# MIT-SPARK/TEASER-plusplus

Measured on AMD Instinct MI355X. Metric: registrations/sec at N=10000 correspondences, 95% outliers, higher is better.
Workload: dtype bf16x3-split MFMA + f32 filter with FP64 fix-up for K1 (bitmap bit-identical to FP64); f64 estimators

## Files before the change

teaser-plusplus_amd/csrc/kernels_graph.hip:

```cpp
#include <algorithm>
#include <utility>
#include <vector>

#include <cstdio>
#include <cstdlib>

#include "internal.h"
#include "fixup_item.h"
#include "fixup_regions.h"
#include "k1_consts.h"
#include "wave_utils.h"

namespace thip {

struct EdgeConst {
  double beta;
  double beta2;
  double m2beta2;
  double beta4;
  double s_hat;
};

__device__ __forceinline__ bool tim_edge_exact(double ax, double ay, double az, double bx,
                                               double by, double bz, double beta) {
// ... 316 lines not shown
    const float na = (float)na_d, nb = (float)nb_d;
    int ra, rb, pa, pb;
    k1c::xy_shifts(kexp, &ra, &rb, &pa, &pb);
    const float fra = (float)k1c::pow2_d(-ra), frb = (float)k1c::pow2_d(-rb), fpa = (float)k1c::pow2_d(-pa);
    const unsigned short P = f16_bits((float)k1c::pow2_d(-pb));
    unsigned short A[32], B[32];
    for (int k = 0; k < 32; ++k) A[k] = B[k] = 0;
    const float cs[3] = {sx, sy, sz}, cd[3] = {dx, dy, dz};
    float h, m, l;
    for (int c = 0; c < 3; ++c) {
      f16_split3(cs[c] * fra, &h, &m, &l);
      A[3 * c] = f16_bits(h); A[3 * c + 1] = A[3 * c]; A[3 * c + 2] = f16_bits(m);
      f16_split3(cs[c] * frb, &h, &m, &l);
      B[3 * c] = f16_bits(2.0f * h); B[3 * c + 1] = f16_bits(2.0f * m); B[3 * c + 2] = B[3 * c];
      f16_split3(cd[c] * fra, &h, &m, &l);
      A[16 + 3 * c] = f16_bits(h); A[16 + 3 * c + 1] = A[16 + 3 * c]; A[16 + 3 * c + 2] = f16_bits(m);
      f16_split3(cd[c] * frb, &h, &m, &l);
      B[16 + 3 * c] = f16_bits(-2.0f * h); B[16 + 3 * c + 1] = f16_bits(-2.0f * m); B[16 + 3 * c + 2] = B[16 + 3 * c];
    }
    f16_split3(na * fpa, &h, &m, &l);
    A[9] = f16_bits(-h); A[10] = f16_bits(-m); A[11] = f16_bits(-l); B[9] = P; B[10] = P; B[11] = P;
    B[12] = A[9]; B[13] = A[10]; B[14] = A[11]; A[12] = P; A[13] = P; A[14] = P;
    f16_split3(nb * fpa, &h, &m, &l);
    A[25] = f16_bits(h); A[26] = f16_bits(m); A[27] = f16_bits(l); B[25] = P; B[26] = P; B[27] = P;
    B[28] = A[25]; B[29] = A[26]; B[30] = A[27]; A[28] = P; A[29] = P; A[30] = P;
    A[31] = 0xb400;
    B[31] = 0x3c00;
    TimOperandTile2* tile = ops + d.w_off + (ip >> 6);
    const int gq = (ip >> 5) & 1, cc = ip & 31;
    for (int mf = 0; mf < kTimRowOperands; ++mf)
      for (int hh = 0; hh < 2; ++hh) {
        const unsigned short* pa = A + 16 * mf + 8 * hh;
        tile->a[gq][mf][hh][cc] = make_uint4(pa[0] | ((unsigned int)pa[1] << 16), pa[2] | ((unsigned int)pa[3] << 16),
                                             pa[4] | ((unsigned int)pa[5] << 16), pa[6] | ((unsigned int)pa[7] << 16));
        if (mf >= kTimColOperands) continue;
        const unsigned short* pb = B + 16 * mf + 8 * hh;
        tile->b[gq][mf][hh][cc] = make_uint4(pb[0] | ((unsigned int)pb[1] << 16), pb[2] | ((unsigned int)pb[3] << 16),
                                             pb[4] | ((unsigned int)pb[5] << 16), pb[6] | ((unsigned int)pb[7] << 16));
      }
    mx = na > nb ? na : nb;
    if (!(mx == mx)) mx = INFINITY;
    if (ip < d.n) deg[d.pt_off + ip] = 0;
  }
  for (int o = 32; o > 0; o >>= 1) {
    const float t = __shfl_xor(mx, o, 64);
    mx = t > mx ? t : mx;
  }
  if ((threadIdx.x & 63) == 0 && mx > 0.f) atomicMax(&prep[blockIdx.y].r2_bits, __float_as_uint(mx));
}

#ifdef TEASER_K1_LAB
struct TimOperandTile3 {
  uint4 a[2][3][2][32];
  uint4 b[2][2][2][32];
};
__global__ __launch_bounds__(256) void tim_prep_pack3_kernel(const ProbDesc* __restrict__ descs,
                                                             const double* __restrict__ src,
                                                             const double* __restrict__ dst,
                                                             TimPrep* __restrict__ prep,
                                                             TimOperandTile3* __restrict__ ops,
                                                             int32_t* __restrict__ deg, double beta) {
  const ProbDesc d = descs[blockIdx.y];
  const int ip = blockIdx.x * 256 + threadIdx.x;
  float mx = 0.f;
  if (ip < d.W * 64 && d.n > 0) {
    double g;
    int kexp;
    k1c::scale(beta, &g, &kexp);
    const int i = min(ip, d.n - 1);
    const TimPrep* pr = prep + blockIdx.y;
    const int sh = k1c::norm_shift(prep_half_extent(pr));
    kexp += 2 * sh;
    g *= k1c::pow2_d(sh);
    const double* a = src + 3 * (d.pt_off + i);
    const double* b = dst + 3 * (d.pt_off + i);
    const float sx = (float)((a[0] - prep_centre(pr, 0, 0)) * g), sy = (float)((a[1] - prep_centre(pr, 0, 1)) * g),
                sz = (float)((a[2] - prep_centre(pr, 0, 2)) * g);
    const float dx = (float)((b[0] - prep_centre(pr, 1, 0)) * g), dy = (float)((b[1] - prep_centre(pr, 1, 1)) * g),
                dz = (float)((b[2] - prep_centre(pr, 1, 2)) * g);
    const double na_d = ((double)sx * sx + (double)sy * sy) + (double)sz * sz;
    const double nb_d = ((double)dx * dx + (double)dy * dy) + (double)dz * dz;
    const float na = (float)na_d, nb = (float)nb_d;
    const double beta2s = k1c::pow2_d(kexp - 2);
    const float kappa = (float)k1c::pow2_d(kexp);
    const float delta_row = (float)(nb_d - na_d - beta2s);
    const float delta_col = (float)(nb_d - na_d);
    unsigned short A[48], B[32];
    for (int k = 0; k < 48; ++k) A[k] = 0;
    for (int k = 0; k < 32; ++k) B[k] = 0;
    const float cs[3] = {sx, sy, sz}, cd[3] = {dx, dy, dz};
    const unsigned short one = 0x3c00;
    float h, m, l;
    for (int c = 0; c < 3; ++c) {
      f16_split3(cs[c], &h, &m, &l);
      B[3 * c] = f16_bits(2.0f * h); B[3 * c + 1] = f16_bits(2.0f * m); B[3 * c + 2] = B[3 * c];
      A[3 * c] = f16_bits(h); A[3 * c + 1] = A[3 * c]; A[3 * c + 2] = f16_bits(m);
      A[32 + 3 * c] = f16_bits(kappa * h); A[32 + 3 * c + 1] = A[32 + 3 * c]; A[32 + 3 * c + 2] = f16_bits(kappa * m);
      f16_split3(cd[c], &h, &m, &l);
      B[16 + 3 * c] = f16_bits(-2.0f * h); B[16 + 3 * c + 1] = f16_bits(-2.0f * m); B[16 + 3 * c + 2] = B[16 + 3 * c];
      A[16 + 3 * c] = f16_bits(h); A[16 + 3 * c + 1] = A[16 + 3 * c]; A[16 + 3 * c + 2] = f16_bits(m);
    }
    f16_split3(na, &h, &m, &l);
    B[9] = f16_bits(-h); B[10] = f16_bits(-m);
    A[32 + 9] = f16_bits(kappa); A[32 + 10] = A[32 + 9];
    B[11] = one; B[12] = one; B[13] = one;
    B[14] = f16_bits(kappa); B[15] = B[14];
    A[32 + 14] = f16_bits(-h); A[32 + 15] = f16_bits(-m);
    f16_split3(delta_row, &h, &m, &l);
    A[11] = f16_bits(h); A[12] = f16_bits(m); A[13] = f16_bits(l);
    f16_split3(delta_col, &h, &m, &l);
    A[25] = one; A[26] = one; A[27] = one; B[25] = f16_bits(h); B[26] = f16_bits(m); B[27] = f16_bits(l);
    TimOperandTile3* tile = ops + d.w_off + (ip >> 6);
    const int gq = (ip >> 5) & 1, cc = ip & 31;
    for (int mf = 0; mf < 3; ++mf)
      for (int hh = 0; hh < 2; ++hh) {
        const unsigned short* pa = A + 16 * mf + 8 * hh;
        tile->a[gq][mf][hh][cc] = make_uint4(pa[0] | ((unsigned int)pa[1] << 16), pa[2] | ((unsigned int)pa[3] << 16),
                                             pa[4] | ((unsigned int)pa[5] << 16), pa[6] | ((unsigned int)pa[7] << 16));
        if (mf >= kTimColOperands) continue;
        const unsigned short* pb = B + 16 * mf + 8 * hh;
        tile->b[gq][mf][hh][cc] = make_uint4(pb[0] | ((unsigned int)pb[1] << 16), pb[2] | ((unsigned int)pb[3] << 16),
                                             pb[4] | ((unsigned int)pb[5] << 16), pb[6] | ((unsigned int)pb[7] << 16));
      }
    mx = na > nb ? na : nb;
    if (!(mx == mx)) mx = INFINITY;
    if (ip < d.n) deg[d.pt_off + ip] = 0;
  }
  for (int o = 32; o > 0; o >>= 1) {
    const float t = __shfl_xor(mx, o, 64);
    mx = t > mx ? t : mx;
  }
  if ((threadIdx.x & 63) == 0 && mx > 0.f) atomicMax(&prep[blockIdx.y].r2_bits, __float_as_uint(mx));
}
#endif

__global__ void tim_prep_consts_kernel(TimPrep* __restrict__ prep, int batch, double beta) {
  const int p = blockIdx.x * blockDim.x + threadIdx.x;
  if (p >= batch) return;
  const k1c::ConstsXY c = k1c::consts_xy(beta, k1c::norm_shift(prep_half_extent(prep + p)), prep[p].r2_bits);
  prep[p].band_c = c.C;
  prep[p].use_mfma = c.use_mfma;
}
#ifdef TEASER_K1_LAB
__global__ void tim_prep_consts3_kernel(TimPrep* __restrict__ prep, int batch, double beta) {
  const int p = blockIdx.x * blockDim.x + threadIdx.x;
  if (p >= batch) return;
  const k1c::Consts c = k1c::consts(beta, k1c::norm_shift(prep_half_extent(prep + p)), prep[p].r2_bits);
  prep[p].band_c = c.C;
  prep[p].use_mfma = c.use_mfma;
}
#endif


constexpr bool kK1Pipe = false, kK1Plain = true;
constexpr int kK1Chunks = 1, kK1Occ = 3;

constexpr int kK1NoStore = 1, kK1Rebuild = 2;
template <bool PIPE, bool PLAIN, int OCC, int CHUNKS, bool LOWER, bool UW3 = false, int NS = 0>
__global__ __launch_bounds__(256, OCC) void tim_graph_mfma3_kernel(
    const ProbDesc* __restrict__ descs, const double* __restrict__ src,
    const double* __restrict__ dst, const void* __restrict__ ops, const TimPrep* __restrict__ prep,
    uint64_t* __restrict__ bitmap, double beta, int gyr,
    unsigned long long* __restrict__ work, unsigned int* __restrict__ work_count,
    ProbState* __restrict__ states, int32_t* __restrict__ deg, unsigned long long* __restrict__ regions, int Tmax,
    int rb_open, int nlb_arg) {
  static_assert(NS == 0 || (NS == kK1NoStore && !LOWER) || (NS == kK1Rebuild && LOWER), "store modes");
  if constexpr (NS == kK1Rebuild) {
    if ((rb_open && states[blockIdx.y].deg_closed) || !prep[blockIdx.y].use_mfma) return;
  }
  const ProbDesc d = descs[blockIdx.y];
  const int n = d.n, W = d.W;
  const int T = W, S = bm_stride(W);
  int lb = (int)blockIdx.x;
  const int nlb = NS == kK1Rebuild ? nlb_arg : (int)gridDim.x;
  do {
  int Ig, X;
  fxr::decode_block(lb, nlb, gyr, CHUNKS, &Ig, &X);
  constexpr int kBlockColTiles = kMfmaColTiles * CHUNKS;
  const int I0 = Ig * kMfmaRowTiles, Jbase = X * kBlockColTiles;
  auto region_of = [&](int wv, int chunk) -> unsigned long long* {
    if constexpr (NS == kK1Rebuild) return nullptr;
    const int Iw = I0 + wv, Xc = X * CHUNKS + chunk;
    return fxr::is_cell(Iw, Xc, Tmax) ? regions + fxr::region_offset((int)blockIdx.y, Tmax, Iw, Xc) : nullptr;
  };
  auto zero_regions = [&]() {
    if ((threadIdx.x & 63) < CHUNKS) {
      unsigned long long* r = region_of((int)(threadIdx.x >> 6), (int)(threadIdx.x & 63));
      if (r) r[0] = 0ull;
    }
  };
  if (I0 >= T || Jbase >= T || Jbase + kBlockColTiles - 1 < I0) {
    zero_regions();
    continue;
  }
  const int lane = threadIdx.x & 63;
  const int wave = __builtin_amdgcn_readfirstlane(threadIdx.x >> 6);
  const int I = I0 + wave;

  const double* __restrict__ ps = src + 3 * d.pt_off;
  const double* __restrict__ pd = dst + 3 * d.pt_off;
  uint64_t* __restrict__ bm = bitmap + d.bm_off;
  __shared__ __attribute__((aligned(16))) uint64_t lds_own[kMfmaRowTiles][64][kMfmaColTiles + 1];
  static_assert(sizeof(lds_own[0]) >= sizeof(double) * 64 * 6 && sizeof(lds_own[0]) >= 8 * kWorkBuf, "aliased buffers");
  __shared__ __attribute__((aligned(16))) uint64_t lds_tr[kMfmaColTiles][64][kMfmaRowTiles];
  constexpr int kRowOps = UW3 ? 3 : kTimRowOperands;
  constexpr int kTileBytes = 2 * (kRowOps + kTimColOperands) * 1024, kColBase = 2 * kRowOps * 1024;
  static_assert(UW3 || (kTileBytes == (int)sizeof(TimOperandTile2) && kColBase == (int)offsetof(TimOperandTile2, b)), "tile layout");
  const char* __restrict__ qt = reinterpret_cast<const char*>(ops) + (size_t)d.w_off * kTileBytes;
  const int h = lane >> 5, c = lane & 31;
  typedef unsigned int u32x4 __attribute__((ext_vector_type(4)));
  const __amdgpu_buffer_rsrc_t q_rsrc = __builtin_amdgcn_make_buffer_rsrc(
      (void*)qt, 0, (int)((unsigned int)T * (unsigned int)kTileBytes), 0x00020000);
  auto load_op = [&](int tile, int side, int g, int m) -> uint4 {
    const int soff = tile * kTileBytes + (side ? kColBase + (g * kTimColOperands + m) * 1024 : (g * kRowOps + m) * 1024);
    const u32x4 v = __builtin_amdgcn_raw_buffer_load_b128(q_rsrc, lane * 16, soff, 0);
    return make_uint4(v.x, v.y, v.z, v.w);
  };
  f16x8 ar[2][kRowOps];
  {
    const int It = min(I, T - 1);
    for (int rt = 0; rt < 2; ++rt)
      for (int m = 0; m < kRowOps; ++m) ar[rt][m] = __builtin_bit_cast(f16x8, load_op(It, 0, rt, m));
  }
  const bool rowvalid = I < T;
  const uint64_t rowmask = !rowvalid ? 0ull : (n - I * 64 >= 64) ? ~0ull : ((1ull << (n - I * 64)) - 1ull);
  const int Jfirst = max(Jbase, I), Jend = min(Jbase + kBlockColTiles, T);
  uint4 bX[kTimColOperands], bY[kTimColOperands];
  {
    const int Jf = min(Jfirst, T - 1);
    for (int m = 0; m < kTimColOperands; ++m) bX[m] = load_op(Jf, 1, 0, m);
    if (PIPE)
      for (int m = 0; m < kTimColOperands; ++m) bY[m] = load_op(Jf, 1, 1, m);
  }
  const TimPrep pr = prep[blockIdx.y];
  if (!pr.use_mfma) {
    EdgeConst kc;
    kc.beta = beta;
    kc.beta2 = beta * beta;
    kc.m2beta2 = -2.0 * kc.beta2;
    kc.beta4 = kc.beta2 * kc.beta2;
    kc.s_hat = 1.0;
    if (I < T)
      for (int jb = Jbase; jb < Jbase + kBlockColTiles; jb += kColTilesPerWave)
        if (!(jb + kColTilesPerWave - 1 < I || jb >= T))
          tim_wave_fp64<0>(ps, pd, bm, n, W, I, jb, kc, reinterpret_cast<double*>(&lds_own[wave][0][0]));
    zero_regions();
    continue;
  }
  const __amdgpu_buffer_rsrc_t deg_rsrc = __builtin_amdgcn_make_buffer_rsrc(
      (void*)(deg + d.pt_off), 0, (int)((unsigned int)n * 4u), 0x00020000);
  const __amdgpu_buffer_rsrc_t bm_rsrc = __builtin_amdgcn_make_buffer_rsrc(
      (void*)bm, 0, (int)((unsigned int)n * (unsigned int)S * 8u), 0x00020000);
  int degacc = 0;
  const int cq = c - 4 * h;
  const int selfq = (cq >= 0 && (cq & 4) == 0) ? ((cq & 3) | ((cq >> 3) << 2)) : -1;
  unsigned int flags = 0;
  const float thr = pr.band_c;

  struct Acc {
    f32x16 U, W;
  };
  static_assert(!(UW3 && PIPE), "the three-MFMA lab variant has the flat schedule only");
  auto mf = [&](Acc& a, const f16x8(&arow)[kRowOps], const uint4(&b)[kTimColOperands]) {
    f32x16 z;
    for (int k = 0; k < 16; ++k) z[k] = 0.f;
    a.W = __builtin_amdgcn_mfma_f32_32x32x16_f16(arow[0], __builtin_bit_cast(f16x8, b[0]), z, 0, 0, 0);
    a.U = __builtin_amdgcn_mfma_f32_32x32x16_f16(arow[1], __builtin_bit_cast(f16x8, b[1]), a.W, 0, 0, 0);
  };
  auto epi = [&](const Acc& a, bool self_tile) -> unsigned int {
    unsigned int colbits = 0;
    float m = INFINITY;
#pragma unroll
    for (int qp = 7; qp >= 0; --qp) {
      float d0, d1;
      if (PLAIN) {
        d0 = __builtin_fmaf(a.U[2 * qp], a.U[2 * qp], a.W[2 * qp]);
        d1 = __builtin_fmaf(a.U[2 * qp + 1], a.U[2 * qp + 1], a.W[2 * qp + 1]);
      } else {
        const f32x2 u2 = {a.U[2 * qp], a.U[2 * qp + 1]}, w2 = {a.W[2 * qp], a.W[2 * qp + 1]};
        const f32x2 d2 = __builtin_elementwise_fma(u2, u2, w2);
        d0 = d2.x;
        d1 = d2.y;
      }
      float v0 = __builtin_fabsf(d0), v1 = __builtin_fabsf(d1);
      if (self_tile) {
        v0 = (selfq == 2 * qp) ? INFINITY : v0;
        v1 = (selfq == 2 * qp + 1) ? INFINITY : v1;
      }
      m = __builtin_fminf(__builtin_fminf(m, v0), v1);
      colbits = __builtin_amdgcn_alignbit(colbits, __float_as_uint(d1), (qp & 1) ? 27 : 31);
      colbits = __builtin_amdgcn_alignbit(colbits, __float_as_uint(d0), 31);
    }
    asm("v_cmp_nlt_f32_e32 vcc, %2, %1\n\tv_addc_co_u32_e32 %0, vcc, %0, %0, vcc" : "+v"(flags) : "v"(m), "s"(thr) : "vcc");
    return colbits;
  };
  const unsigned int sel16 = (lane & 16) ? 0x03020706u : 0x01000504u;
  auto finish_tile = [&](const int J, const bool diag, const unsigned int (&tr)[2][2]) {
    const int j0 = J * 64;
    unsigned int tw[2], ow[2];
#pragma unroll
    for (int rt = 0; rt < 2; ++rt) {
      const auto r = __builtin_amdgcn_permlane32_swap(tr[0][rt], tr[1][rt], false, false);
      tw[rt] = merge_gap_bytes(r[0], r[1]);
      unsigned int x;
      {
        const auto sw = __builtin_amdgcn_permlane16_swap(tw[rt], tw[rt], false, false);
        x = __builtin_amdgcn_perm(sw[0], sw[1], sel16);
      }
#pragma unroll
      for (int st = 1; st < 5; ++st) {
        const int j = 16 >> st;
        unsigned int p;
        switch (st) {
          case 1: p = __builtin_amdgcn_update_dpp(0u, x, 0x128, 0xf, 0xf, true); break;
          case 2:
            p = __builtin_amdgcn_update_dpp(0u, x, 0x141, 0xf, 0xf, true);
            p = __builtin_amdgcn_update_dpp(0u, p, 0x1b, 0xf, 0xf, true);
            break;
          case 3: p = __builtin_amdgcn_update_dpp(0u, x, 0x4e, 0xf, 0xf, true); break;
          default: p = __builtin_amdgcn_update_dpp(0u, x, 0xb1, 0xf, 0xf, true); break;
        }
        const bool up = (lane & j) != 0;
        const unsigned int shifted = __builtin_amdgcn_alignbit(p, p, up ? j : 32 - j);
        const unsigned int km[5] = {0x0000FFFFu, 0x00FF00FFu, 0x0F0F0F0Fu, 0x33333333u, 0x55555555u};
        const unsigned int keep = up ? ~km[st] : km[st];
        x = bit_select(keep, x, shifted);
      }
      ow[rt] = x;
    }
    const auto ro = __builtin_amdgcn_permlane32_swap(ow[0], ow[1], false, false);
    uint64_t ownw = ((uint64_t)ro[1] << 32) | ro[0];
    const uint64_t trw = ((uint64_t)tw[1] << 32) | tw[0];
    const uint64_t colmask = (n - j0 >= 64) ? ~0ull : ((1ull << (n - j0)) - 1ull);
    ownw &= colmask;
    if (diag) ownw &= ~(1ull << lane);
    if (NS != kK1NoStore || diag) lds_own[wave][lane][(J - Jbase) & (kMfmaColTiles - 1)] = ownw;
    degacc += __builtin_popcountll(ownw);
    const uint64_t trw_out = diag ? 0ull : (trw & rowmask);
    lds_tr[(J - Jbase) & (kMfmaColTiles - 1)][lane][wave] = trw_out;
  };

  auto body_flat = [&](const int J, auto diag_tag) {
    constexpr bool DIAG = decltype(diag_tag)::value;
    unsigned int tr[2][2];
#pragma unroll
    for (int ct = 0; ct < 2; ++ct) {
      const f16x8 b0 = __builtin_bit_cast(f16x8, bX[0]), b1 = __builtin_bit_cast(f16x8, bX[1]);
      const int Jn = (ct == 0 || J + 1 >= Jend) ? J : J + 1, gn = ct ^ 1;
      f32x16 z;
      for (int k = 0; k < 16; ++k) z[k] = 0.f;
      Acc acc[2];
      __builtin_amdgcn_s_setprio(2);
      if constexpr (UW3) {
        acc[0].U = __builtin_amdgcn_mfma_f32_32x32x16_f16(ar[0][0], b0, z, 0, 0, 0);
        __builtin_amdgcn_sched_barrier(0);
        acc[1].U = __builtin_amdgcn_mfma_f32_32x32x16_f16(ar[1][0], b0, z, 0, 0, 0);
        __builtin_amdgcn_sched_barrier(0);
        acc[0].W = __builtin_amdgcn_mfma_f32_32x32x16_f16(ar[0][kRowOps - 1], b0, z, 0, 0, 0);
        __builtin_amdgcn_sched_barrier(0);
        acc[1].W = __builtin_amdgcn_mfma_f32_32x32x16_f16(ar[1][kRowOps - 1], b0, z, 0, 0, 0);
      } else {
        acc[0].W = __builtin_amdgcn_mfma_f32_32x32x16_f16(ar[0][0], b0, z, 0, 0, 0);
        __builtin_amdgcn_sched_barrier(0);
        acc[1].W = __builtin_amdgcn_mfma_f32_32x32x16_f16(ar[1][0], b0, z, 0, 0, 0);
      }
      __builtin_amdgcn_sched_barrier(0);
      bX[0] = load_op(Jn, 1, gn, 0);
      __builtin_amdgcn_sched_barrier(0);
      acc[0].U = __builtin_amdgcn_mfma_f32_32x32x16_f16(ar[0][1], b1, UW3 ? acc[0].U : acc[0].W, 0, 0, 0);
      __builtin_amdgcn_sched_barrier(0);
      acc[1].U = __builtin_amdgcn_mfma_f32_32x32x16_f16(ar[1][1], b1, UW3 ? acc[1].U : acc[1].W, 0, 0, 0);
      __builtin_amdgcn_sched_barrier(0);
      bX[1] = load_op(Jn, 1, gn, 1);
      __builtin_amdgcn_s_setprio(0);
      __builtin_amdgcn_sched_barrier(0);
#pragma unroll
      for (int rt = 0; rt < 2; ++rt) tr[ct][rt] = epi(acc[rt], DIAG && ct == rt);
    }
    finish_tile(J, DIAG, tr);
  };

  Acc accA, accB;
#define TIM_K1_INTERLEAVE(N)                                                              \
  __builtin_amdgcn_sched_group_barrier(0x008, 1, 0);                                      \
  __builtin_amdgcn_sched_group_barrier(0x002, N, 0);                                      \
  __builtin_amdgcn_sched_group_barrier(0x008, 1, 0);                                      \
  __builtin_amdgcn_sched_group_barrier(0x002, N, 0);                                      \
  __builtin_amdgcn_sched_group_barrier(0x008, 1, 0);                                      \
  __builtin_amdgcn_sched_group_barrier(0x002, N, 0);                                      \
  __builtin_amdgcn_sched_group_barrier(0x008, 1, 0);                                      \
  __builtin_amdgcn_sched_group_barrier(0x002, N, 0)
  constexpr int kEpiShare = PLAIN ? 13 : 9;
  auto body_pipe = [&](const int J, auto diag_tag) {
    constexpr bool DIAG = decltype(diag_tag)::value;
    const int Jn = min(J + 1, Jend - 1);
    unsigned int tr[2][2];
    mf(accB, ar[1], bX);
    tr[0][0] = epi(accA, DIAG);
    TIM_K1_INTERLEAVE(kEpiShare);
    __builtin_amdgcn_sched_barrier(0);
    for (int m = 0; m < kTimColOperands; ++m) bX[m] = load_op(Jn, 1, 0, m);
    mf(accA, ar[0], bY);
    tr[0][1] = epi(accB, false);
    __builtin_amdgcn_sched_group_barrier(0x020, kTimColOperands, 0);
    TIM_K1_INTERLEAVE(kEpiShare);
    __builtin_amdgcn_sched_barrier(0);
    mf(accB, ar[1], bY);
    tr[1][0] = epi(accA, false);
    TIM_K1_INTERLEAVE(kEpiShare);
    __builtin_amdgcn_sched_barrier(0);
    for (int m = 0; m < kTimColOperands; ++m) bY[m] = load_op(Jn, 1, 1, m);
    mf(accA, ar[0], bX);
    tr[1][1] = epi(accB, DIAG);
    finish_tile(J, DIAG, tr);
    __builtin_amdgcn_sched_group_barrier(0x020, kTimColOperands, 0);
    TIM_K1_INTERLEAVE(kEpiShare + 16);
    __builtin_amdgcn_sched_barrier(0);
  };

#undef TIM_K1_INTERLEAVE
  unsigned long long* wbuf = reinterpret_cast<unsigned long long*>(&lds_own[wave][0][0]);
  bool primed = false;
#pragma nounroll
  for (int chunk = 0; chunk < CHUNKS; ++chunk) {
    const int Jc0 = Jbase + chunk * kMfmaColTiles, Jc1 = min(Jc0 + kMfmaColTiles, Jend);
    unsigned long long* const region = region_of(wave, chunk);
    if (Jc0 >= Jend) {
      if (lane == 0 && region) region[0] = 0ull;
      continue;
    }
    const int Ja = rowvalid ? max(Jc0, Jfirst) : Jc1;
    if (Ja < Jc1) {
      int J = Ja;
      if (PIPE) {
        if (!primed) {
          mf(accA, ar[0], bX);
          __builtin_amdgcn_sched_barrier(0);
          primed = true;
        }
        if (J == I) {
          body_pipe(J, std::true_type());
          ++J;
        }
#pragma nounroll
        for (; J < Jc1; ++J) body_pipe(J, std::false_type());
      } else {
        if (J == I) {
          body_flat(J, std::true_type());
          ++J;
        }
#pragma nounroll
        for (; J < Jc1; ++J) body_flat(J, std::false_type());
      }
    }
    const int nact = max(Jc1 - Ja, 0);
    {
      __syncthreads();
#pragma unroll
      for (int it = 0; it < (kMfmaColTiles * 64) / 256; ++it) {
        const int idx = it * 256 + (int)threadIdx.x, Jr = idx >> 6, r = idx & 63, J = Jc0 + Jr, j = J * 64 + r;
        const uint4 lo = *reinterpret_cast<const uint4*>(&lds_tr[Jr][r][0]);
        const uint4 hi = *reinterpret_cast<const uint4*>(&lds_tr[Jr][r][2]);
        const bool rowok = J < Jc1 && j < n;
        const unsigned int base = ((unsigned int)j * (unsigned int)S + (unsigned int)I0) * 8u;
        if (Jc0 > I0 + 3 && I0 + 3 < T) {
          const int cnt = (__builtin_popcount(lo.x) + __builtin_popcount(lo.y)) + (__builtin_popcount(lo.z) + __builtin_popcount(lo.w)) +
                          (__builtin_popcount(hi.x) + __builtin_popcount(hi.y)) + (__builtin_popcount(hi.z) + __builtin_popcount(hi.w));
          if (LOWER) {
            __builtin_amdgcn_raw_buffer_store_b128(u32x4{lo.x, lo.y, lo.z, lo.w}, bm_rsrc, rowok ? base : kOobOffset, 0, 0);
            __builtin_amdgcn_raw_buffer_store_b128(u32x4{hi.x, hi.y, hi.z, hi.w}, bm_rsrc, rowok ? base + 16u : kOobOffset, 0, 0);
          }
          __builtin_amdgcn_raw_ptr_buffer_atomic_add_i32(cnt, deg_rsrc, (rowok && cnt) ? (unsigned int)j * 4u : kOobOffset, 0, 0);
          continue;
        }
        bool ok[4];
        for (int k = 0; k < 4; ++k) ok[k] = rowok && I0 + k < T && I0 + k < J;
        const unsigned int w32[8] = {lo.x, lo.y, lo.z, lo.w, hi.x, hi.y, hi.z, hi.w};
        int cnt = 0;
        for (int k = 0; k < 4; ++k) cnt += ok[k] ? __builtin_popcount(w32[2 * k]) + __builtin_popcount(w32[2 * k + 1]) : 0;
        if (!LOWER) {
        } else if (ok[3]) {
          __builtin_amdgcn_raw_buffer_store_b128(u32x4{lo.x, lo.y, lo.z, lo.w}, bm_rsrc, base, 0, 0);
          __builtin_amdgcn_raw_buffer_store_b128(u32x4{hi.x, hi.y, hi.z, hi.w}, bm_rsrc, base + 16u, 0, 0);
        } else {
          for (int k = 0; k < 3; ++k)
            __builtin_amdgcn_raw_buffer_store_b64(u32x2{w32[2 * k], w32[2 * k + 1]}, bm_rsrc,
                                                  ok[k] ? base + 8u * k : kOobOffset, 0, 0);
        }
        __builtin_amdgcn_raw_ptr_buffer_atomic_add_i32(cnt, deg_rsrc, cnt ? (unsigned int)j * 4u : kOobOffset, 0, 0);
      }
      if (CHUNKS > 1) __syncthreads();
    }
    if (NS == kK1NoStore) {
      if (Ja == I && Ja < Jc1) {
        const uint64_t w = lds_own[wave][lane][(I - Jbase) & (kMfmaColTiles - 1)];
        __builtin_amdgcn_raw_buffer_store_b64(u32x2{(unsigned int)w, (unsigned int)(w >> 32)}, bm_rsrc,
                                              I * 64 + lane < n ? ((unsigned int)(I * 64 + lane) * (unsigned int)S + (unsigned int)I) * 8u : kOobOffset,
                                              0, 0);
      }
    } else if (nact > 0) {
      const int kk = lane & 7, J = Jc0 + kk;
      const bool pad = J >= T, colok = (J >= Ja && J < Jc1) || pad;
      const unsigned int off0 = ((unsigned int)(I * 64 + (lane >> 3)) * (unsigned int)S + (unsigned int)J) * 8u;
#pragma unroll
      for (int it = 0; it < 8; ++it) {
        const int r = it * 8 + (lane >> 3);
        const uint64_t w = pad ? 0ull : lds_own[wave][r][kk];
        __builtin_amdgcn_raw_buffer_store_b64(u32x2{(unsigned int)w, (unsigned int)(w >> 32)}, bm_rsrc,
                                              (colok && I * 64 + r < n) ? off0 + (unsigned int)it * 64u * (unsigned int)S : kOobOffset,
                                              0, 0);
      }
    }
    int wcount = 0;
    if constexpr (NS != kK1Rebuild) {
      unsigned int vf = flags;
      if (I * 64 + 4 * h >= n) vf &= ~0xAAAAAAAAu;
      if (I * 64 + 32 + 4 * h >= n) vf &= ~0x55555555u;
      if (T - 1 >= Ja && T - 1 < Jc1 && (n & 63)) {
        const int sh = 4 * (Jc1 - T);
        if ((T - 1) * 64 + c >= n) vf &= ~(0xCu << sh);
        if ((T - 1) * 64 + 32 + c >= n) vf &= ~(0x3u << sh);
      }
      if (__builtin_amdgcn_ballot_w64(vf != 0u) != 0ull) {
        const int mine = __builtin_popcount(vf);
        int base = 0, total = 0;
#pragma unroll
        for (int bit = 0; bit < 6; ++bit) {
          const uint64_t m = __builtin_amdgcn_ballot_w64(((mine >> bit) & 1) != 0);
          base += (int)__builtin_amdgcn_mbcnt_hi((unsigned int)(m >> 32), __builtin_amdgcn_mbcnt_lo((unsigned int)m, 0u)) << bit;
          total += __builtin_popcountll(m) << bit;
        }
        if (total > kWorkBuf) {
          if (lane == 0) states[blockIdx.y].k1_overflow = 1;
        } else {
          int kk = base;
#pragma nounroll
          while (vf) {
            const int pos = 31 - __builtin_clz(vf);
            vf &= ~(1u << pos);
            const int J = Ja + (nact - 1 - (pos >> 2));
            const int ct = ((pos >> 1) & 1) ^ 1, rt = (pos & 1) ^ 1;
            const unsigned int rowp = (unsigned int)(I * 64 + 32 * rt + 4 * h);
            const unsigned int colp = (unsigned int)(J * 64 + 32 * ct + c);
            const uint64_t tword = lds_tr[(J - Jbase) & (kMfmaColTiles - 1)][32 * ct + c][wave];
            wbuf[kk++] = fxi::pack(rowp, colp, fxi::gather_bits(tword, rt, h));
          }
          wcount = total;
        }
      }
    }
    flags = 0;
    if constexpr (NS != kK1Rebuild) {
      const int nreg = !region ? 0 : (wcount < kRegionItems ? wcount : kRegionItems);
      if (lane == 0 && region) region[0] = (unsigned long long)nreg;
      if (lane < nreg) region[1 + lane] = wbuf[lane];
      if (wcount > nreg) {
        const int extra = wcount - nreg;
        unsigned int base = 0;
        if (lane == 0) base = atomicAdd(work_count + blockIdx.y, (unsigned int)extra);
        base = __builtin_amdgcn_readfirstlane(base);
        if (base + (unsigned int)extra > pr.seg_cap) {
          if (lane == 0) states[blockIdx.y].k1_overflow = 1;
        } else {
          unsigned long long* seg = work + (((size_t)pr.seg_off_hi << 32) | (size_t)pr.seg_off_lo);
#pragma nounroll
          for (int k2i = lane; k2i < extra; k2i += 64) seg[base + k2i] = wbuf[nreg + k2i];
        }
      }
    }
  }
  if (rowvalid)
    __builtin_amdgcn_raw_ptr_buffer_atomic_add_i32(degacc, deg_rsrc, (unsigned int)(I * 64 + lane) * 4u, 0, 0);
  } while (NS == kK1Rebuild && (__syncthreads(), (lb += (int)gridDim.x) < nlb));
}

constexpr int kFixUpper = 1;
template <bool NOSTORE>
__global__ __launch_bounds__(256) void tim_fixup_group_kernel(const ProbDesc* __restrict__ descs, int batch,
                                                              const double* __restrict__ src,
                                                              const double* __restrict__ dst,
                                                              uint64_t* __restrict__ bitmap, double beta,
                                                              unsigned long long* __restrict__ work,
                                                              const unsigned int* __restrict__ work_count,
                                                              ProbState* __restrict__ states,
                                                              int32_t* __restrict__ deg,
                                                              unsigned long long* __restrict__ regions,
                                                              int Tmax,
                                                              const TimPrep* __restrict__ prep, int mode) {
  TAIL_WAVE_PRIO();
  constexpr bool nostore = NOSTORE;
  const bool upper = nostore || (mode & kFixUpper) != 0;
  const int prob = blockIdx.y;
  const unsigned int total = work_count[prob];
  const TimPrep tpr = prep[prob];
  const unsigned int cap = tpr.seg_cap;
  const ProbDesc d = descs[prob];
  const int n = d.n, W = d.W, S = bm_stride(W);
  if (total > cap) {
    const int64_t words = (int64_t)n * S;
    uint64_t* bm = bitmap + d.bm_off;
    for (int64_t w = (int64_t)blockIdx.x * 256 + threadIdx.x; w < words; w += (int64_t)gridDim.x * 256) bm[w] = 0;
    if (blockIdx.x == 0 && threadIdx.x == 0) states[prob].k1_overflow = 1;
    return;
  }
  int32_t* dg = deg + d.pt_off;
  if (!tpr.use_mfma) {
    const uint64_t* bm = bitmap + d.bm_off;
    const int lane = threadIdx.x & 63;
    for (int row = blockIdx.x * 4 + (threadIdx.x >> 6); row < n; row += gridDim.x * 4) {
      const uint64_t* r = bm + (int64_t)row * S;
      int c = 0;
      for (int w = lane; w < W; w += 64) c += __popcll(r[w]);
      c = wave_sum_i(c);
      if (lane == 0) dg[row] = c;
    }
    return;
  }
  const double* ps = src + 3 * d.pt_off;
  const double* pd = dst + 3 * d.pt_off;
  unsigned int* bm32 = reinterpret_cast<unsigned int*>(bitmap + d.bm_off);
  EdgeConst kc;
  kc.beta = beta;
  kc.beta2 = beta * beta;
  kc.m2beta2 = -2.0 * kc.beta2;
  kc.beta4 = kc.beta2 * kc.beta2;
  kc.s_hat = 1.0;
  const int lane = threadIdx.x & 63, q = lane & 15, sub = lane >> 4, wave = threadIdx.x >> 6;
  const int rq = (q & 3) + 8 * (q >> 2);
  __shared__ double row_pts[4][64][6];
  __shared__ __attribute__((aligned(16))) double col_pts[4][64][6];
  auto resolve = [&](unsigned long long it, bool valid, auto staged, int tile, int slot, unsigned long long* home) {
    constexpr bool STAGED = decltype(staged)::value;
    const bool live = valid;
    int r = fxi::row0(it) + rq, col = fxi::col(it);
    valid = valid && r < n && col < n && r != col;
    r = valid ? r : (STAGED ? tile * 64 : 0);
    col = valid ? col : 0;
    double sx, sy, sz, dx, dy, dz, cx, cy, cz, ex, ey, ez;
    if (STAGED) {
      const double* rp = row_pts[wave][r & 63];
      sx = rp[0]; sy = rp[1]; sz = rp[2]; dx = rp[3]; dy = rp[4]; dz = rp[5];
      const double* cp = col_pts[wave][slot];
      cx = cp[0]; cy = cp[1]; cz = cp[2]; ex = cp[3]; ey = cp[4]; ez = cp[5];
    } else {
      sx = ps[3 * r]; sy = ps[3 * r + 1]; sz = ps[3 * r + 2];
      dx = pd[3 * r]; dy = pd[3 * r + 1]; dz = pd[3 * r + 2];
      cx = ps[3 * col]; cy = ps[3 * col + 1]; cz = ps[3 * col + 2];
      ex = pd[3 * col]; ey = pd[3 * col + 1]; ez = pd[3 * col + 2];
    }
    unsigned int* wp = bm32 + 2 * ((int64_t)r * S + (col >> 6)) + ((col >> 5) & 1);
    const unsigned int bit = 1u << (col & 31);
    const bool offdiag = (r >> 6) != (col >> 6);
    bool prov;
    if ((STAGED || nostore) && offdiag) {
      prov = fxi::bit(it, q);
    } else {
      prov = (*wp & bit) != 0u;
    }
    const double ax = cx - sx, ay = cy - sy, az = cz - sz, bx = ex - dx, by = ey - dy, bz = ez - dz;
    bool unc, shortp;
    bool e = tim_edge_fast(ax, ay, az, bx, by, bz, kc, &unc, &shortp);
    e |= shortp;
    if (unc) e = tim_edge_exact(ax, ay, az, bx, by, bz, beta);
    if constexpr (nostore) {
      const uint64_t em = __builtin_amdgcn_ballot_w64(valid && e);
      if (q == 0 && live) *home = fxi::pack((unsigned int)fxi::row0(it), (unsigned int)fxi::col(it), (unsigned int)(em >> (16 * sub)) & 0xffffu);
    }
    if (!valid || prov == e) return;
    if (!nostore || !offdiag) atomicXor(wp, bit);
    atomicAdd(dg + r, e ? 1 : -1);
    if (offdiag) {
      if (!upper) atomicXor(bm32 + 2 * ((int64_t)col * S + (r >> 6)) + ((r >> 5) & 1), 1u << (r & 31));
      atomicAdd(dg + col, e ? 1 : -1);
    }
  };
  __shared__ unsigned long long queue[4][2 * kRegionWords];
  static_assert(kRegionWords == 64, "one region = one 64-lane load");
  __shared__ unsigned short qsrc[nostore ? 4 : 1][nostore ? 2 * kRegionWords : 1];
  const int T = W, nch = fxr::n_chunks(T);
  auto round = [&](int cnt, int tile, unsigned long long* run) {
    if (lane < cnt) {
      const int col = min(fxi::col(queue[wave][lane]), n - 1);
      double* cp = col_pts[wave][lane];
      const double c0 = ps[3 * col], c1 = ps[3 * col + 1], c2 = ps[3 * col + 2];
      const double e0 = pd[3 * col], e1 = pd[3 * col + 1], e2 = pd[3 * col + 2];
      cp[0] = c0; cp[1] = c1; cp[2] = c2; cp[3] = e0; cp[4] = e1; cp[5] = e2;
    }
    __builtin_amdgcn_fence(__ATOMIC_ACQ_REL, "wavefront");
#pragma nounroll
    for (int base = 0; base < cnt; base += 4) {
      const int k = base + sub;
      resolve(queue[wave][k], k < cnt, std::true_type(), tile, k, nostore ? run + qsrc[nostore ? wave : 0][nostore ? k : 0] : nullptr);
    }
    __builtin_amdgcn_fence(__ATOMIC_ACQ_REL, "wavefront");
  };
  const int wv = blockIdx.x * 4 + wave, nwv = gridDim.x * 4, npairs = (T + 1) >> 1;
  for (int pi = wv; pi < npairs; pi += nwv) {
    for (int side = 0; side < 2; ++side) {
      const int tile = side ? T - 1 - pi : pi;
      if (side && tile == pi) break;
      {
        const int pr = min(tile * 64 + lane, n - 1);
        double* rp = row_pts[wave][lane];
        rp[0] = ps[3 * pr]; rp[1] = ps[3 * pr + 1]; rp[2] = ps[3 * pr + 2];
        rp[3] = pd[3 * pr]; rp[4] = pd[3 * pr + 1]; rp[5] = pd[3 * pr + 2];
      }
      const int Xc0 = fxr::first_chunk(tile);
      unsigned long long* reg = regions + fxr::region_offset(prob, Tmax, tile, Xc0);
      int qn = 0;
      unsigned long long mine = reg[lane];
      for (int Xc = Xc0; Xc < nch; ++Xc) {
        const unsigned long long cur = mine;
        if (Xc + 1 < nch) mine = reg[(size_t)(Xc + 1 - Xc0) * kRegionWords + lane];
        const int cnt = min((int)__builtin_amdgcn_readfirstlane((unsigned int)cur), kRegionItems);
        if (cnt <= 0) continue;
        if (lane >= 1 && lane <= cnt) {
          queue[wave][qn + lane - 1] = cur;
          if constexpr (nostore) qsrc[wave][qn + lane - 1] = (unsigned short)((Xc - Xc0) * kRegionWords + lane);
        }
        qn += cnt;
        if (qn >= kRegionWords) {
          __builtin_amdgcn_fence(__ATOMIC_ACQ_REL, "wavefront");
          round(kRegionWords, tile, reg);
          qn -= kRegionWords;
          const unsigned long long moved = queue[wave][kRegionWords + lane];
          unsigned short moved_src = 0;
// ... 182 lines not shown
static int64_t tim_region_words(int max_n) { return fxr::arena_words((max_n + 63) / 64); }

static int64_t tim_segment_items(int n) {
  const int64_t seg = std::max<int64_t>((int64_t)n * (n - 1) / 2 / 256, 1 << 16);
  return std::min<int64_t>(seg, 0x7fffffffll);
}
int64_t tim_work_items(const int32_t* n, int batch) {
  int64_t segs = 0;
  int max_n = 0;
  for (int b = 0; b < batch; ++b) {
    segs += tim_segment_items(n[b]);
    max_n = std::max(max_n, n[b]);
  }
  return segs + tim_region_words(max_n) * std::max(batch, 1);
}
int64_t tim_prep_fill_segments(void* host_prep, const int32_t* n, int batch) {
  TimPrep* pr = reinterpret_cast<TimPrep*>(host_prep);
  int64_t off = 0;
  for (int b = 0; b < batch; ++b) {
    const int64_t seg = tim_segment_items(n[b]);
    pr[b].seg_off_lo = (unsigned int)((uint64_t)off & 0xffffffffu);
    pr[b].seg_off_hi = (unsigned int)((uint64_t)off >> 32);
    pr[b].seg_cap = (unsigned int)seg;
    off += seg;
  }
  return off;
}

int tim_probe_worklist(const void* d_prep, const void* d_work, int64_t work_cap, int batch, int max_n,
                       unsigned long long* regions_out, int64_t* stride_words, int64_t* used_regions,
                       unsigned int* seg_counts) {
  const int64_t reg_words = tim_region_words(max_n);
  *stride_words = reg_words;
  *used_regions = fxr::cells((max_n + 63) / 64);
  if (!regions_out) return 0;
  const unsigned long long* regions = reinterpret_cast<const unsigned long long*>(d_work) + (work_cap - reg_words * (int64_t)batch);
  hipError_t e = hipMemcpy(regions_out, regions, (size_t)reg_words * (size_t)batch * 8, hipMemcpyDeviceToHost);
  if (e == hipSuccess && seg_counts)
    e = hipMemcpy(seg_counts, reinterpret_cast<const char*>(d_prep) + sizeof(TimPrep) * (size_t)batch, 4 * (size_t)batch,
                  hipMemcpyDeviceToHost);
  return (int)e;
}

#ifdef TEASER_K1_LAB
struct K1Variant { int pipe, plain, chunks, occ4, uw3; };
static K1Variant k1_lab_variant() {
  const char* ev = getenv("TEASER_K1_VARIANT");
  const int v = ev ? atoi(ev) : 0;
  K1Variant k;
  k.uw3 = (v / 10000) % 10 != 0;
  k.occ4 = (v / 1000) % 10 != 0;
  k.pipe = v % 10 != 0;
  k.plain = (v / 10) % 10 != 0;
  k.chunks = 1 << ((v / 100) % 10);
  return k;
}
#endif

void launch_tim_graph_mfma(hipStream_t s, int phase, const ProbDesc* d_desc, int batch, int max_n,
                           int64_t total_tiles, const double* d_src, const double* d_dst,
                           void* d_pk, void* d_prep, void* d_work, int64_t work_cap,
                           uint64_t* d_bitmap, ProbState* d_state, int32_t* d_deg, double noise_bound,
                           double cbar2) {
  if (batch <= 0 || max_n <= 0) return;
  (void)total_tiles;
  const int T = (max_n + 63) / 64;
  if (phase == kTimMirror || phase == kTimMirrorOpen) {
    if (T < 2) return;
    const int waves = T * ((T + kMirrorRun - 1) / kMirrorRun);
    hipLaunchKernelGGL(tim_mirror_lower_kernel, dim3((unsigned)std::min(64, (waves + 3) / 4), batch), dim3(256), 0, s, d_desc,
                       d_bitmap, d_state, phase == kTimMirrorOpen ? 1 : 0);
    return;
  }
  const double beta = 2 * noise_bound * sqrt(cbar2);
  if (phase == kTimClosurePairs) {
    int32_t* counters = reinterpret_cast<int32_t*>(d_prep);
    launch_degree_closure_order(s, d_desc, batch, d_deg, d_state, d_pk, counters);
    const ClosurePools cp = degree_closure_pools(d_pk, batch);
    hipLaunchKernelGGL(tim_closure_pairs_kernel, dim3(degree_closure_wgs(batch), batch), dim3(256), 0, s, d_desc, d_src, d_dst,
                       cp.part, cp.keys, counters, beta);
    return;
  }
#ifdef TEASER_K1_LAB
  const bool upper = false, nostore = false;
  if (phase == kTimRebuild || phase == kTimRebuildOpen) return;
#else
  const bool upper = (phase & kTimUpperOnly) != 0;
  const bool nostore = (phase & kTimNoStore) != 0;
#endif
  phase &= ~(kTimUpperOnly | kTimNoStore);
  TimPrep* prep = reinterpret_cast<TimPrep*>(d_prep);
  unsigned long long* work = reinterpret_cast<unsigned long long*>(d_work);
  unsigned int* work_count = reinterpret_cast<unsigned int*>(reinterpret_cast<char*>(d_prep) +
                                                            sizeof(TimPrep) * (size_t)batch);
  const int64_t reg_words = tim_region_words(max_n);
  unsigned long long* regions = work + (work_cap - reg_words * (int64_t)batch);
#ifdef TEASER_K1_LAB
  const K1Variant lab = k1_lab_variant();
#endif
  if (phase == 0) {
    hipLaunchKernelGGL(tim_prep_bbox_kernel, dim3((max_n + 1023) / 1024, batch), dim3(256), 0, s, d_desc,
                       d_src, d_dst, prep);
#ifdef TEASER_K1_LAB
    if (lab.uw3) {
      hipLaunchKernelGGL(tim_prep_pack3_kernel, dim3((T * 64 + 255) / 256, batch), dim3(256), 0, s, d_desc, d_src,
                         d_dst, prep, reinterpret_cast<TimOperandTile3*>(d_pk), d_deg, beta);
      hipLaunchKernelGGL(tim_prep_consts3_kernel, dim3((batch + 63) / 64), dim3(64), 0, s, prep, batch, beta);
      return;
    }
#endif
    hipLaunchKernelGGL(tim_prep_pack2_kernel, dim3((T * 64 + 255) / 256, batch), dim3(256), 0, s, d_desc, d_src,
                       d_dst, prep, reinterpret_cast<TimOperandTile2*>(d_pk), d_deg, beta);
    hipLaunchKernelGGL(tim_prep_consts_kernel, dim3((batch + 63) / 64), dim3(64), 0, s, prep, batch, beta);
  } else if (phase == 1) {
    const int gyr = (T + kMfmaRowTiles - 1) / kMfmaRowTiles;
#define TIM_K1_LAUNCH(PIPE, PLAIN, CHUNKS) TIM_K1_LAUNCH_OCC(PIPE, PLAIN, kK1Occ, CHUNKS, true)
#define TIM_K1_LAUNCH_OCC(PIPE, PLAIN, OCC, CHUNKS, ...)                                                                       \
  hipLaunchKernelGGL((tim_graph_mfma3_kernel<PIPE, PLAIN, OCC, CHUNKS, __VA_ARGS__>), dim3(tim_mfma_blocks(T, CHUNKS), batch), \
                     dim3(256), 0, s, d_desc, d_src, d_dst, (const void*)d_pk, prep, d_bitmap, beta, gyr, work, work_count,    \
                     d_state, d_deg, regions, T, 0, 0)
#ifdef TEASER_K1_LAB
#define TIM_K1_LAB_CASE(PIPE, PLAIN)                             \
  if (lab.pipe == (PIPE ? 1 : 0) && lab.plain == (PLAIN ? 1 : 0)) { \
    if (lab.chunks == 1) { TIM_K1_LAUNCH(PIPE, PLAIN, 1); }      \
    else if (lab.chunks == 2) { TIM_K1_LAUNCH(PIPE, PLAIN, 2); } \
    else { TIM_K1_LAUNCH(PIPE, PLAIN, 4); }                      \
  }
    if (lab.uw3) {
      if (lab.plain) { TIM_K1_LAUNCH_OCC(false, true, kK1Occ, 1, true, true); } else { TIM_K1_LAUNCH_OCC(false, false, kK1Occ, 1, true, true); }
    } else if (lab.occ4) {
      if (lab.plain) { TIM_K1_LAUNCH_OCC(false, true, 4, 1, true); } else { TIM_K1_LAUNCH_OCC(false, false, 4, 1, true); }
    } else {
      TIM_K1_LAB_CASE(false, false)
      TIM_K1_LAB_CASE(false, true)
      TIM_K1_LAB_CASE(true, false)
      TIM_K1_LAB_CASE(true, true)
    }
#undef TIM_K1_LAB_CASE
#else
    if (nostore) {
      TIM_K1_LAUNCH_OCC(kK1Pipe, kK1Plain, kK1Occ, kK1Chunks, false, false, kK1NoStore);
    } else if (upper) {
      TIM_K1_LAUNCH_OCC(kK1Pipe, kK1Plain, kK1Occ, kK1Chunks, false);
    } else {
      TIM_K1_LAUNCH(kK1Pipe, kK1Plain, kK1Chunks);
    }
#endif
#undef TIM_K1_LAUNCH
#undef TIM_K1_LAUNCH_OCC
#ifndef TEASER_K1_LAB
  } else if (phase == kTimRebuild || phase == kTimRebuildOpen) {
    const int gyr = (T + kMfmaRowTiles - 1) / kMfmaRowTiles, nlb = tim_mfma_blocks(T, kK1Chunks);
    const int open_only = phase == kTimRebuildOpen ? 1 : 0;
    hipLaunchKernelGGL((tim_graph_mfma3_kernel<kK1Pipe, kK1Plain, 2, kK1Chunks, true, false, kK1Rebuild>),
                       dim3(open_only ? std::min(64, nlb) : nlb, batch), dim3(256), 0, s, d_desc, d_src, d_dst,
                       (const void*)d_pk, prep, d_bitmap, beta, gyr, work, work_count, d_state, d_deg, regions, T, open_only, nlb);
    hipLaunchKernelGGL(tim_fixup_replay_kernel, dim3((unsigned)std::max(4, ((T + 3) / 4 + 1) / 2), batch), dim3(256), 0, s,
                       d_desc, d_bitmap, work, work_count, d_state, regions, T, prep, open_only);
#endif
  } else {
    const int64_t forced_wgs = setting(S_FIXUP_WGS);
    const int64_t fix_wgs = forced_wgs > 0 ? forced_wgs : ((T + 1) / 2 + 3) / 4;
    const dim3 fix_grid((unsigned)std::max<int64_t>(4, fix_wgs), batch);
    if (nostore)
      hipLaunchKernelGGL(tim_fixup_group_kernel<true>, fix_grid, dim3(256), 0, s, d_desc, batch, d_src, d_dst, d_bitmap, beta,
                         work, work_count, d_state, d_deg, regions, T, prep, 0);
    else
      hipLaunchKernelGGL(tim_fixup_group_kernel<false>, fix_grid, dim3(256), 0, s, d_desc, batch, d_src, d_dst, d_bitmap, beta,
                         work, work_count, d_state, d_deg, regions, T, prep, upper ? kFixUpper : 0);
  }
}

__global__ __launch_bounds__(256) void degree_kernel(const ProbDesc* __restrict__ descs,
                                                     const uint64_t* __restrict__ bitmap,
                                                     int32_t* __restrict__ deg) {
  const ProbDesc d = descs[blockIdx.y];
  const int lane = threadIdx.x & 63;
  for (int row = blockIdx.x * 4 + (threadIdx.x >> 6); row < d.n; row += gridDim.x * 4) {
    const uint64_t* r = bitmap + d.bm_off + (int64_t)row * bm_stride(d.W);
    int c = 0;
    for (int w = lane; w < d.W; w += 64) c += __popcll(r[w]);
    c = wave_sum_i(c);
    if (lane == 0) deg[d.pt_off + row] = c;
  }
}

void launch_degrees(hipStream_t s, const ProbDesc* d_desc, int batch, int max_n,
                    const uint64_t* d_bitmap, int32_t* d_deg, ProbState* d_state) {
  if (batch <= 0 || max_n <= 0) return;
  dim3 grid((max_n + 3) / 4, batch);
  hipLaunchKernelGGL(degree_kernel, grid, dim3(256), 0, s, d_desc, d_bitmap, d_deg);
}

__global__ __launch_bounds__(256) void trims_kernel(const double* __restrict__ src,
                                                    const double* __restrict__ dst, int n,
                                                    double beta, double* __restrict__ raw,
                                                    double* __restrict__ alpha) {
  const int i = blockIdx.x;
  if (i >= n - 1) return;
  const int64_t seg = (int64_t)i * n - (int64_t)i * (i + 1) / 2;
  const double six = src[3 * i], siy = src[3 * i + 1], siz = src[3 * i + 2];
  const double dix = dst[3 * i], diy = dst[3 * i + 1], diz = dst[3 * i + 2];
  for (int j = i + 1 + threadIdx.x; j < n; j += 256) {
    const double ax = src[3 * j] - six, ay = src[3 * j + 1] - siy, az = src[3 * j + 2] - siz;
    const double bx = dst[3 * j] - dix, by = dst[3 * j + 1] - diy, bz = dst[3 * j + 2] - diz;
    const double v1 = __builtin_sqrt((ax * ax + ay * ay) + az * az);
    const double v2 = __builtin_sqrt((bx * bx + by * by) + bz * bz);
    const int64_t k = seg + (j - i - 1);
    raw[k] = v2 / v1;
    alpha[k] = beta * (1.0 / v1);
  }
}

void launch_trims(hipStream_t s, const double* d_src, const double* d_dst, int n, double beta,
                  double* d_raw, double* d_alpha) {
  if (n < 2) return;
  hipLaunchKernelGGL(trims_kernel, dim3(n - 1), dim3(256), 0, s, d_src, d_dst, n, beta, d_raw,
                     d_alpha);
}

__global__ void fill_identity_clique_kernel(const ProbDesc* __restrict__ descs,
                                            int32_t* __restrict__ clique,
                                            ProbState* __restrict__ states) {
  const ProbDesc d = descs[blockIdx.y];
  const int i = blockIdx.x * blockDim.x + threadIdx.x;
  if (i < d.n) clique[d.pt_off + i] = i;
  if (i == 0) {
    ProbState* st = states + blockIdx.y;
    st->lb = d.n;
    st->clique_size = d.n;
    st->proven = 1;
    st->peel_done = 1;
  }
}

void launch_fill_identity_clique(hipStream_t s, const ProbDesc* d_desc, int batch, int max_n,
                                 int32_t* d_clique, ProbState* d_state) {
  if (batch <= 0) return;
  const int bx = max_n > 0 ? (max_n + 255) / 256 : 1;
  hipLaunchKernelGGL(fill_identity_clique_kernel, dim3(bx, batch), dim3(256), 0, s, d_desc,
                     d_clique, d_state);
}

}
```

Before: 124,500.

## Compact open-problem rebuild grid into slots that search for still-open problems

In the open-only rebuild phase the grid is now a small number of y-slots instead of one y per batch problem. Each block uses a wave ballot to find the ord-th problem that is still open and MFMA-eligible, then strides to later open problems once its own tiles are done. The x dimension now covers all blocks of a problem instead of being capped at 64. This avoids launching and early-exiting many blocks for closed problems and gives more parallelism per open problem, at the cost of repeated ballot scans over the batch and reduced cross-problem parallelism when many problems stay open.

```diff
diff --git a/teaser-plusplus_amd/csrc/kernels_graph.hip b/teaser-plusplus_amd/csrc/kernels_graph.hip
--- a/teaser-plusplus_amd/csrc/kernels_graph.hip
+++ b/teaser-plusplus_amd/csrc/kernels_graph.hip
@@ -492,8 +492,40 @@
 #endif
 
 
+__device__ __forceinline__ int k1_rebuild_find_open(const ProbState* __restrict__ states, const TimPrep* __restrict__ prep,
+                                                    const int batch, int ord) {
+  const int ln = (int)(threadIdx.x & 63);
+  for (int base = 0; base < batch; base += 64) {
+    const int b = base + ln;
+    const bool open = b < batch && !states[b].deg_closed && prep[b].use_mfma;
+    uint64_t m = __builtin_amdgcn_ballot_w64(open);
+    const int cnt = __builtin_popcountll(m);
+    if (ord < cnt) {
+      for (int k = 0; k < ord; ++k) m &= m - 1ull;
+      return base + (int)__builtin_ctzll(m);
+    }
+    ord -= cnt;
+  }
+  return -1;
+}
+__device__ __forceinline__ bool k1_rebuild_next(int& lb, const int nlb, int& ord, unsigned int& pb, const int rb_open,
+                                                const ProbState* __restrict__ states, const TimPrep* __restrict__ prep,
+                                                const ProbDesc* __restrict__ descs, ProbDesc& d, int& n, int& W, int& T, int& S) {
+  if ((lb += (int)gridDim.x) < nlb) return true;
+  if (!rb_open) return false;
+  ord += (int)gridDim.y;
+  const int found = k1_rebuild_find_open(states, prep, rb_open, ord);
+  if (found < 0) return false;
+  pb = (unsigned int)found;
+  lb = (int)blockIdx.x;
+  d = descs[pb];
+  n = d.n, W = d.W, T = W, S = bm_stride(W);
+  return true;
+}
+
 constexpr bool kK1Pipe = false, kK1Plain = true;
 constexpr int kK1Chunks = 1, kK1Occ = 3;
+constexpr int kRebuildOpenSlots = 2;
 
 constexpr int kK1NoStore = 1, kK1Rebuild = 2;
 template <bool PIPE, bool PLAIN, int OCC, int CHUNKS, bool LOWER, bool UW3 = false, int NS = 0>
@@ -505,12 +537,20 @@
     ProbState* __restrict__ states, int32_t* __restrict__ deg, unsigned long long* __restrict__ regions, int Tmax,
     int rb_open, int nlb_arg) {
   static_assert(NS == 0 || (NS == kK1NoStore && !LOWER) || (NS == kK1Rebuild && LOWER), "store modes");
+  unsigned int pb = blockIdx.y;
+  int ord = (int)blockIdx.y;
   if constexpr (NS == kK1Rebuild) {
-    if ((rb_open && states[blockIdx.y].deg_closed) || !prep[blockIdx.y].use_mfma) return;
-  }
-  const ProbDesc d = descs[blockIdx.y];
-  const int n = d.n, W = d.W;
-  const int T = W, S = bm_stride(W);
+    if (rb_open) {
+      const int found = k1_rebuild_find_open(states, prep, rb_open, ord);
+      if (found < 0) return;
+      pb = (unsigned int)found;
+    } else if (!prep[pb].use_mfma) {
+      return;
+    }
+  }
+  ProbDesc d = descs[pb];
+  int n = d.n, W = d.W;
+  int T = W, S = bm_stride(W);
   int lb = (int)blockIdx.x;
   const int nlb = NS == kK1Rebuild ? nlb_arg : (int)gridDim.x;
   do {
@@ -521,7 +561,7 @@
   auto region_of = [&](int wv, int chunk) -> unsigned long long* {
     if constexpr (NS == kK1Rebuild) return nullptr;
     const int Iw = I0 + wv, Xc = X * CHUNKS + chunk;
-    return fxr::is_cell(Iw, Xc, Tmax) ? regions + fxr::region_offset((int)blockIdx.y, Tmax, Iw, Xc) : nullptr;
+    return fxr::is_cell(Iw, Xc, Tmax) ? regions + fxr::region_offset((int)pb, Tmax, Iw, Xc) : nullptr;
   };
   auto zero_regions = [&]() {
     if ((threadIdx.x & 63) < CHUNKS) {
@@ -572,7 +612,7 @@
     if (PIPE)
       for (int m = 0; m < kTimColOperands; ++m) bY[m] = load_op(Jf, 1, 1, m);
   }
-  const TimPrep pr = prep[blockIdx.y];
+  const TimPrep pr = prep[pb];
   if (!pr.use_mfma) {
     EdgeConst kc;
     kc.beta = beta;
@@ -871,7 +911,7 @@
           total += __builtin_popcountll(m) << bit;
         }
         if (total > kWorkBuf) {
-          if (lane == 0) states[blockIdx.y].k1_overflow = 1;
+          if (lane == 0) states[pb].k1_overflow = 1;
         } else {
           int kk = base;
 #pragma nounroll
@@ -897,10 +937,10 @@
       if (wcount > nreg) {
         const int extra = wcount - nreg;
         unsigned int base = 0;
-        if (lane == 0) base = atomicAdd(work_count + blockIdx.y, (unsigned int)extra);
+        if (lane == 0) base = atomicAdd(work_count + pb, (unsigned int)extra);
         base = __builtin_amdgcn_readfirstlane(base);
         if (base + (unsigned int)extra > pr.seg_cap) {
-          if (lane == 0) states[blockIdx.y].k1_overflow = 1;
+          if (lane == 0) states[pb].k1_overflow = 1;
         } else {
           unsigned long long* seg = work + (((size_t)pr.seg_off_hi << 32) | (size_t)pr.seg_off_lo);
 #pragma nounroll
@@ -911,7 +951,8 @@
   }
   if (rowvalid)
     __builtin_amdgcn_raw_ptr_buffer_atomic_add_i32(degacc, deg_rsrc, (unsigned int)(I * 64 + lane) * 4u, 0, 0);
-  } while (NS == kK1Rebuild && (__syncthreads(), (lb += (int)gridDim.x) < nlb));
+  } while (NS == kK1Rebuild &&
+           (__syncthreads(), k1_rebuild_next(lb, nlb, ord, pb, rb_open, states, prep, descs, d, n, W, T, S)));
 }
 
 constexpr int kFixUpper = 1;
@@ -1400,9 +1441,11 @@
   } else if (phase == kTimRebuild || phase == kTimRebuildOpen) {
     const int gyr = (T + kMfmaRowTiles - 1) / kMfmaRowTiles, nlb = tim_mfma_blocks(T, kK1Chunks);
     const int open_only = phase == kTimRebuildOpen ? 1 : 0;
+    const dim3 rb_grid = open_only ? dim3(nlb, kRebuildOpenSlots) : dim3(nlb, batch);
     hipLaunchKernelGGL((tim_graph_mfma3_kernel<kK1Pipe, kK1Plain, 2, kK1Chunks, true, false, kK1Rebuild>),
-                       dim3(open_only ? std::min(64, nlb) : nlb, batch), dim3(256), 0, s, d_desc, d_src, d_dst,
-                       (const void*)d_pk, prep, d_bitmap, beta, gyr, work, work_count, d_state, d_deg, regions, T, open_only, nlb);
+                       rb_grid, dim3(256), 0, s, d_desc, d_src, d_dst,
+                       (const void*)d_pk, prep, d_bitmap, beta, gyr, work, work_count, d_state, d_deg, regions, T,
+                       open_only ? batch : 0, nlb);
     hipLaunchKernelGGL(tim_fixup_replay_kernel, dim3((unsigned)std::max(4, ((T + 3) / 4 + 1) / 2), batch), dim3(256), 0, s,
                        d_desc, d_bitmap, work, work_count, d_state, regions, T, prep, open_only);
 #endif
```

Result: faster. 128,900 (median of 6 runs) (+3.5%).
